# mit-han-lab/duo-attention

Measured on NVIDIA H100. Metric: decode tok/s @512K ctx (+ prefill tok/s @128K in `prefill`), Llama-3-8B, DuoAttention 50% retrieval heads, higher is better.
Workload: dtype bf16

## Files before the change

duo_attention_b200/_C.py:

```python
from __future__ import annotations

import ctypes as C
import os

_HERE = os.path.dirname(os.path.abspath(__file__))
LIB_PATH = os.environ.get("DUO_B200_LIB") or os.path.join(_HERE, "csrc", "libduo_b200.so")

DUO_OK, DUO_EINVAL, DUO_EOVERFLOW, DUO_ECUDA, DUO_EWORKSPACE = 0, -1, -2, -3, -4
DT_BF16, DT_FP16 = 0, 1
KV_SAME, KV_INT4 = 0, 1
ROPE_NONE, ROPE_HF, ROPE_FP32 = 0, 1, 2
ROPE_SKIP_Q = 0x100
DECODE_MAX_Q = 16
DECODE_MAX_Q_INT4 = 8
RAGGED_MAX_BATCH = 64

SYMBOLS = [
    "duo_layer_create", "duo_layer_destroy", "duo_workspace_bytes", "duo_rope_append", "duo_attention",
    "duo_attention_mma", "duo_decode_fused", "duo_decode_ragged", "duo_ragged_workspace_bytes",
    "duo_decode_ragged_int4", "duo_ragged_int4_workspace_bytes", "duo_layer_create_pooled", "duo_decode_ragged_pooled",
    "duo_ragged_state_advance", "duo_state_advance", "duo_state_set", "duo_stream_commit", "duo_quant_int4", "duo_dequant_int4", "duo_dequant_int4_bf16", "duo_add_rmsnorm", "duo_silu_mul",
    "duo_attention_partial", "duo_merge_partials", "duo_attention_seq", "duo_decode_fused_seq",
    "duo_attention_seq_int4", "duo_decode_fused_seq_int4",
    "duo_seqcomm_data_bytes", "duo_seqcomm_flag_bytes", "duo_seqcomm_create", "duo_seqcomm_destroy", "duo_seq_merge",
    "duo_comm_data_bytes", "duo_comm_flag_bytes", "duo_comm_create", "duo_comm_destroy", "duo_allreduce_add_rmsnorm",
    "duo_last_error_string", "duo_version",
]


class LayerDesc(C.Structure):
    _fields_ = [
        ("full_k", C.c_void_p), ("full_v", C.c_void_p), ("ring_k", C.c_void_p), ("ring_v", C.c_void_p),
        ("full_k_scale", C.c_void_p), ("full_k_zero", C.c_void_p), ("full_v_scale", C.c_void_p),
        ("full_v_zero", C.c_void_p), ("ring_k_scale", C.c_void_p), ("ring_k_zero", C.c_void_p),
        ("ring_v_scale", C.c_void_p), ("ring_v_zero", C.c_void_p),
        ("full_cap", C.c_int64),
        ("batch", C.c_int32), ("n_full", C.c_int32), ("n_stream", C.c_int32), ("group", C.c_int32),
        ("head_dim", C.c_int32), ("sink", C.c_int32), ("recent", C.c_int32), ("stage_cap", C.c_int32),
        ("dtype", C.c_int32), ("kv_format", C.c_int32),
    ]


class CacheState(C.Structure):
    _fields_ = [("full_len", C.c_int64), ("total", C.c_int64), ("lo", C.c_int64), ("device_state", C.c_void_p),
                ("seq_rank", C.c_int32), ("seq_world", C.c_int32), ("seq_block", C.c_int32), ("seq_reserved", C.c_int32)]


class SeqCommDesc(C.Structure):
    _fields_ = [("data", C.c_void_p * 8), ("flags", C.c_void_p * 8), ("local_state", C.c_void_p),
                ("rank", C.c_int32), ("world", C.c_int32), ("max_rows", C.c_int32)]


class CommDesc(C.Structure):
    _fields_ = [("data", C.c_void_p * 8), ("flags", C.c_void_p * 8), ("local_state", C.c_void_p),
# ... 29 lines not shown
        fn = getattr(lib, name)
        fn.argtypes = [vp, C.POINTER(CacheState), vp, i64, vp, i32, f32, vp, sz, vp]
        fn.restype = C.c_int
    lib.duo_decode_fused.argtypes = [vp, C.POINTER(CacheState), vp, i64, vp, vp, i32, vp, i32, f32, vp, sz, vp]
    lib.duo_decode_fused.restype = C.c_int
    for name in ("duo_decode_ragged", "duo_decode_ragged_int4"):
        fn = getattr(lib, name)
        fn.argtypes = [vp, vp, i64, vp, i64, vp, vp, i32, vp, i32, f32, vp, sz, vp]
        fn.restype = C.c_int
    lib.duo_decode_ragged_pooled.argtypes = [vp, vp, vp, i64, vp, i64, vp, vp, i32, vp, i32, f32, vp, sz, vp]
    lib.duo_decode_ragged_pooled.restype = C.c_int
    for name in ("duo_ragged_workspace_bytes", "duo_ragged_int4_workspace_bytes"):
        fn = getattr(lib, name)
        fn.argtypes = [i32, i32]
        fn.restype = sz
    lib.duo_ragged_state_advance.argtypes = [vp, i32, i32, i32, i32, vp]
    lib.duo_ragged_state_advance.restype = C.c_int
    lib.duo_state_advance.argtypes = [vp, i32, i32, i32, vp]
    lib.duo_state_advance.restype = C.c_int
    lib.duo_state_set.argtypes = [vp, i64, i64, i64, vp]
    lib.duo_state_set.restype = C.c_int
    lib.duo_stream_commit.argtypes = [vp, C.POINTER(CacheState), i32, vp]
    lib.duo_stream_commit.restype = C.c_int
    lib.duo_quant_int4.argtypes = [vp, i64, i64, vp, vp, vp, vp]
    lib.duo_quant_int4.restype = C.c_int
    for name in ("duo_dequant_int4", "duo_dequant_int4_bf16"):
        fn = getattr(lib, name)
        fn.argtypes = [vp, vp, vp, i64, vp, vp]
        fn.restype = C.c_int
    lib.duo_add_rmsnorm.argtypes = [vp, vp, vp, vp, vp, i64, i32, f32, i32, vp]
    lib.duo_add_rmsnorm.restype = C.c_int
    lib.duo_silu_mul.argtypes = [vp, vp, i64, i32, i32, vp]
    lib.duo_silu_mul.restype = C.c_int
    lib.duo_attention_partial.argtypes = [vp, i64, vp, i64, vp, vp, i32, f32, vp, sz, vp]
    lib.duo_attention_partial.restype = C.c_int
    for name in ("duo_attention_seq", "duo_attention_seq_int4"):
        fn = getattr(lib, name)
        fn.argtypes = [vp, C.POINTER(CacheState), vp, i64, vp, vp, vp, i32, f32, vp, sz, vp]
        fn.restype = C.c_int
    for name in ("duo_decode_fused_seq", "duo_decode_fused_seq_int4"):
        fn = getattr(lib, name)
        fn.argtypes = [vp, C.POINTER(CacheState), vp, i64, vp, vp, i32, vp, vp, vp, f32, vp, sz, vp]
        fn.restype = C.c_int
    lib.duo_seqcomm_data_bytes.argtypes = [i32, i32]
    lib.duo_seqcomm_data_bytes.restype = sz
    lib.duo_seqcomm_flag_bytes.argtypes = [i32, i32]
    lib.duo_seqcomm_flag_bytes.restype = sz
    lib.duo_seqcomm_create.argtypes = [C.POINTER(SeqCommDesc), C.POINTER(vp)]
    lib.duo_seqcomm_create.restype = C.c_int
    lib.duo_seqcomm_destroy.argtypes = [vp]
    lib.duo_seqcomm_destroy.restype = None
    lib.duo_seq_merge.argtypes = [vp, vp, vp, vp, i32, i32, i32, i32, vp]
    lib.duo_seq_merge.restype = C.c_int
    lib.duo_merge_partials.argtypes = [vp, vp, i32, i64, i32, i32, vp, i32, vp]
    lib.duo_merge_partials.restype = C.c_int
    lib.duo_comm_data_bytes.argtypes = [i32, i32, i32, i32]
    lib.duo_comm_data_bytes.restype = sz
    lib.duo_comm_flag_bytes.argtypes = [i32, i32]
    lib.duo_comm_flag_bytes.restype = sz
    lib.duo_comm_create.argtypes = [C.POINTER(CommDesc), C.POINTER(vp)]
    lib.duo_comm_create.restype = C.c_int
    lib.duo_comm_destroy.argtypes = [vp]
    lib.duo_comm_destroy.restype = None
    lib.duo_allreduce_add_rmsnorm.argtypes = [vp, vp, vp, vp, vp, vp, i32, f32, vp]
    lib.duo_allreduce_add_rmsnorm.restype = C.c_int
    lib.duo_last_error_string.argtypes = []
# ... 19 lines not shown
```

duo_attention_b200/csrc/api.cu:

```cuda
#include <cstdarg>
#include <cstdio>
#include <cstdlib>
#include <cstring>
#include <new>

#include "duo_common.cuh"

namespace duo {

int sm_count_current_device() {
  static int sms[64] = {0};
  int dev = 0;
  if (cudaGetDevice(&dev) != cudaSuccess) return 132;
  int& v = sms[dev & 63];
  if (v == 0) {
    int n = 132;
    if (cudaDeviceGetAttribute(&n, cudaDevAttrMultiProcessorCount, dev) != cudaSuccess || n < 1) n = 132;
    v = n;
  }
  return v;
}

static thread_local char g_err[512] = "";

// ... 35 lines not shown
                        float* part_o, float* part_lse, int q_len, float scale, void* workspace, size_t workspace_bytes,
                        cudaStream_t stream);
int launch_decode_fused(const duo_layer* L, const duo_cache_state* st, const void* qkv, long long row_stride,
                        const void* cos, const void* sin, int rope_mode, void* out, int q_len, float scale,
                        void* workspace, size_t workspace_bytes, cudaStream_t stream);
int launch_decode_fused_int4(const duo_layer* L, const duo_cache_state* st, const void* qkv, long long row_stride,
                             const void* cos, const void* sin, int rope_mode, void* out, int q_len, float scale,
                             void* workspace, size_t workspace_bytes, cudaStream_t stream);
int launch_decode_ragged(const duo_layer* L, const long long* row_state, const long long* row_geom, const void* qkv,
                         long long row_stride, const void* cos, const void* sin, int rope_mode, void* out, int q_len,
                         float scale, void* workspace, size_t workspace_bytes, cudaStream_t stream);
size_t ragged_workspace_bytes(int batch, int n_kv);
int launch_decode_ragged_int4(const duo_layer* L, const long long* row_state, const long long* row_geom,
                              const void* qkv, long long row_stride, const void* cos, const void* sin, int rope_mode,
                              void* out, int q_len, float scale, void* workspace, size_t workspace_bytes,
                              cudaStream_t stream);
size_t ragged_int4_workspace_bytes(int batch, int n_kv);
int launch_ragged_state_advance(long long* st, int batch, int n, int sink, int recent, cudaStream_t stream);
int launch_decode_fused_seq(const duo_layer* L, const duo_cache_state* st, const void* qkv, long long row_stride,
                            const void* cos, const void* sin, int rope_mode, void* out, float* part_o, float* part_lse,
                            float scale, void* workspace, size_t workspace_bytes, cudaStream_t stream);
int launch_attn_int4_seq(const duo_layer* L, const duo_cache_state* st, const void* q, long long q_row_stride,
                         void* out, float* part_o, float* part_lse, int q_len, float scale, void* workspace,
                         size_t workspace_bytes, cudaStream_t stream);
int launch_decode_fused_seq_int4(const duo_layer* L, const duo_cache_state* st, const void* qkv, long long row_stride,
                                 const void* cos, const void* sin, int rope_mode, void* out, float* part_o,
                                 float* part_lse, float scale, void* workspace, size_t workspace_bytes,
                                 cudaStream_t stream);
int launch_merge_partials(const float* o_parts, const float* lse_parts, int n_parts, long long tokens, int heads_total,
                          int heads_used, void* out, int dtype, cudaStream_t stream);
int launch_add_rmsnorm(const void* x, const void* residual, const void* weight, void* out_norm, void* out_res,
                       long long rows, int hidden, float eps, int dtype, cudaStream_t stream);
int launch_silu_mul(const void* gate_up, void* out, long long rows, int inter, int dtype, cudaStream_t stream);

typedef CUresult (*EncodeTiledFn)(CUtensorMap*, CUtensorMapDataType, cuuint32_t, void*, const cuuint64_t*,
                                  const cuuint64_t*, const cuuint32_t*, const cuuint32_t*, CUtensorMapInterleave,
                                  CUtensorMapSwizzle, CUtensorMapL2promotion, CUtensorMapFloatOOBfill);

EncodeTiledFn get_encode_fn() {
  static EncodeTiledFn fn = nullptr;
  if (fn) return fn;
  void* p = nullptr;
  cudaDriverEntryPointQueryResult qres;
  cudaError_t e = cudaGetDriverEntryPoint("cuTensorMapEncodeTiled", &p, cudaEnableDefault, &qres);
  if (e != cudaSuccess || qres != cudaDriverEntryPointSuccess || p == nullptr) {
    set_error("cudaGetDriverEntryPoint(cuTensorMapEncodeTiled) failed: %s", cudaGetErrorString(e));
    cudaGetLastError();
    return nullptr;
  }
  fn = reinterpret_cast<EncodeTiledFn>(p);
  return fn;
}

static int encode_kv_map(CUtensorMap* m, void* base, int dtype, long long slots, long long heads, int box_rows) {
  EncodeTiledFn fn = get_encode_fn();
  if (!fn) return DUO_ECUDA;
  cuuint64_t dims[3] = {(cuuint64_t)kHeadDim, (cuuint64_t)slots, (cuuint64_t)heads};
  cuuint64_t strides[2] = {(cuuint64_t)kHeadDim * 2, (cuuint64_t)slots * kHeadDim * 2};
  cuuint32_t box[3] = {64, (cuuint32_t)box_rows, 1};
  cuuint32_t estr[3] = {1, 1, 1};
  CUresult r = fn(m, dtype == DUO_DT_BF16 ? CU_TENSOR_MAP_DATA_TYPE_BFLOAT16 : CU_TENSOR_MAP_DATA_TYPE_FLOAT16, 3, base,
                  dims, strides, box, estr, CU_TENSOR_MAP_INTERLEAVE_NONE, CU_TENSOR_MAP_SWIZZLE_128B,
                  CU_TENSOR_MAP_L2_PROMOTION_L2_256B, CU_TENSOR_MAP_FLOAT_OOB_FILL_NONE);
  if (r != CUDA_SUCCESS) {
    set_error("cuTensorMapEncodeTiled failed with CUresult %d (base=%p slots=%lld heads=%lld)", (int)r, base, slots,
              heads);
// ... 509 lines not shown
}

int duo_merge_partials(const float* o_parts, const float* lse_parts, int32_t n_parts, int64_t tokens,
                       int32_t heads_total, int32_t heads_used, void* out, int32_t dtype, void* stream) {
  if (n_parts < 1 || tokens < 0 || heads_total < 1 || heads_used < 0 || heads_used > heads_total ||
      (tokens > 0 && heads_used > 0 && (!o_parts || !lse_parts || !out)) ||
      (dtype != DUO_DT_BF16 && dtype != DUO_DT_FP16)) {
    set_error("duo_merge_partials: bad argument");
    return DUO_EINVAL;
  }
  return launch_merge_partials(o_parts, lse_parts, n_parts, tokens, heads_total, heads_used, out, dtype,
                               (cudaStream_t)stream);
}

int duo_add_rmsnorm(const void* x, const void* residual, const void* weight, void* out_norm, void* out_res, int64_t rows,
                    int32_t hidden, float eps, int32_t dtype, void* stream) {
  if (rows < 0 || hidden < 8 || hidden % 8 != 0 || hidden > 16384 || (rows > 0 && (!x || !weight || !out_norm)) ||
      (dtype != DUO_DT_BF16 && dtype != DUO_DT_FP16)) {
    set_error("duo_add_rmsnorm: bad argument");
    return DUO_EINVAL;
  }
  return launch_add_rmsnorm(x, residual, weight, out_norm, out_res, rows, hidden, eps, dtype, (cudaStream_t)stream);
}

int duo_silu_mul(const void* gate_up, void* out, int64_t rows, int32_t inter, int32_t dtype, void* stream) {
  if (rows < 0 || inter < 8 || inter % 8 != 0 || (rows > 0 && (!gate_up || !out)) ||
      (dtype != DUO_DT_BF16 && dtype != DUO_DT_FP16)) {
    set_error("duo_silu_mul: bad argument");
    return DUO_EINVAL;
  }
  return launch_silu_mul(gate_up, out, rows, inter, dtype, (cudaStream_t)stream);
}

int duo_dequant_int4(const void* packed, const void* scale, const void* zero, int64_t rows, void* out, void* stream) {
  if (rows < 0 || (rows > 0 && (!packed || !scale || !zero || !out))) {
    set_error("duo_dequant_int4: bad argument");
    return DUO_EINVAL;
  }
  return launch_dequant_int4(packed, scale, zero, rows, out, (cudaStream_t)stream);
}

int duo_dequant_int4_bf16(const void* packed, const void* scale, const void* zero, int64_t rows, void* out,
                          void* stream) {
  if (rows < 0 || (rows > 0 && (!packed || !scale || !zero || !out))) {
    set_error("duo_dequant_int4_bf16: bad argument");
    return DUO_EINVAL;
  }
  return launch_dequant_int4_bf16(packed, scale, zero, rows, out, (cudaStream_t)stream);
}

}
```

duo_attention_b200/csrc/duo_common.cuh:

```cuda
#pragma once
#include <cuda.h>
#include <cuda_bf16.h>
#include <cuda_fp16.h>
#include <cuda_runtime.h>
#include <stdint.h>

#include <algorithm>

#include "../../include/duo_b200.h"

namespace duo {

constexpr int kHeadDim = 128;

void set_error(const char* fmt, ...);
int cuda_fail(cudaError_t e, const char* what);
#define DUO_CUDA_TRY(expr)                                   \
  do {                                                       \
    cudaError_t _e = (expr);                                 \
    if (_e != cudaSuccess) return ::duo::cuda_fail(_e, #expr); \
  } while (0)

struct LayerMaps {
  CUtensorMap full_k64, full_v64;
// ... 632 lines not shown
  const void* cos = nullptr;
  const void* sin = nullptr;
  int rope_mode = DUO_ROPE_NONE;
};

template <typename P>
inline void fill_fused_args(P& p, const FusedArgs& fa) {
  p.cos = fa.cos;
  p.sin = fa.sin;
  p.rope_mode = fa.rope_mode;
  p.k_off = (long long)p.n_q_heads * kHeadDim;
  p.v_off = (long long)(p.n_q_heads + p.n_full + p.n_stream) * kHeadDim;
}

struct KvMaps {
  const CUtensorMap *fk, *fv, *rk, *rv;
};
inline KvMaps kv_maps(const duo_layer* L, bool box128) {
  const LayerMaps& m = L->maps;
  const CUtensorMap* fk = box128 ? &m.full_k128 : &m.full_k64;
  const CUtensorMap* fv = box128 ? &m.full_v128 : &m.full_v64;
  const CUtensorMap* rk = box128 ? &m.ring_k128 : &m.ring_k64;
  const CUtensorMap* rv = box128 ? &m.ring_v128 : &m.ring_v64;
  return {L->has_full_maps ? fk : rk, L->has_full_maps ? fv : rv, L->has_ring_maps ? rk : fk,
          L->has_ring_maps ? rv : fv};
}

template <typename F>
inline int dispatch_dtype(int dtype, F&& f) {
  if (dtype == DUO_DT_BF16) return f(__nv_bfloat16{});
  return f(__half{});
}

}
```

duo_attention_b200/csrc/elementwise.cu:

```cuda
#include "duo_common.cuh"

namespace duo {

template <typename T>
struct EwCvt;
template <>
struct EwCvt<__nv_bfloat16> {
  __device__ static float to_f(__nv_bfloat16 v) { return __bfloat162float(v); }
  __device__ static __nv_bfloat16 from_f(float v) { return __float2bfloat16_rn(v); }
};
template <>
struct EwCvt<__half> {
  __device__ static float to_f(__half v) { return __half2float(v); }
  __device__ static __half from_f(float v) { return __float2half_rn(v); }
};

template <typename T>
struct alignas(16) Vec8 {
  T v[8];
};

template <typename T>
__global__ void __launch_bounds__(256) add_rmsnorm_kernel(const T* __restrict__ x, const T* __restrict__ residual,
                                                          const T* __restrict__ weight, T* __restrict__ out_norm,
                                                          T* __restrict__ out_res, int hidden, float eps) {
  extern __shared__ float s_row[];
  __shared__ float s_part[8];
  const long long row = blockIdx.x;
  const T* xr = x + row * hidden;
  const T* rr = residual ? residual + row * hidden : nullptr;
  float ss = 0.f;
  for (int i = threadIdx.x * 8; i < hidden; i += blockDim.x * 8) {
    Vec8<T> a = *reinterpret_cast<const Vec8<T>*>(xr + i);
    if (rr) {
      const Vec8<T> b = *reinterpret_cast<const Vec8<T>*>(rr + i);
#pragma unroll
      for (int k = 0; k < 8; ++k) a.v[k] = EwCvt<T>::from_f(EwCvt<T>::to_f(b.v[k]) + EwCvt<T>::to_f(a.v[k]));
      if (out_res) *reinterpret_cast<Vec8<T>*>(out_res + row * hidden + i) = a;
    }
#pragma unroll
    for (int k = 0; k < 8; ++k) {
      const float f = EwCvt<T>::to_f(a.v[k]);
      s_row[i + k] = f;
      ss += f * f;
    }
  }
#pragma unroll
  for (int o = 16; o > 0; o >>= 1) ss += __shfl_xor_sync(0xffffffffu, ss, o);
  if ((threadIdx.x & 31) == 0) s_part[threadIdx.x >> 5] = ss;
  __syncthreads();
  float tot = 0.f;
#pragma unroll
  for (int w = 0; w < 8; ++w) tot += (w < (int)(blockDim.x >> 5)) ? s_part[w] : 0.f;
  const float inv = rsqrtf(tot / (float)hidden + eps);
  for (int i = threadIdx.x * 8; i < hidden; i += blockDim.x * 8) {
    const Vec8<T> w = *reinterpret_cast<const Vec8<T>*>(weight + i);
    Vec8<T> o;
#pragma unroll
    for (int k = 0; k < 8; ++k) {
      const T n = EwCvt<T>::from_f(s_row[i + k] * inv);
      o.v[k] = EwCvt<T>::from_f(EwCvt<T>::to_f(w.v[k]) * EwCvt<T>::to_f(n));
    }
    *reinterpret_cast<Vec8<T>*>(out_norm + row * hidden + i) = o;
  }
}

template <typename T>
__global__ void __launch_bounds__(256) silu_mul_kernel(const T* __restrict__ gate_up, T* __restrict__ out, long long rows,
                                                       int inter) {
  const long long per_row = inter / 8;
  const long long idx = (long long)blockIdx.x * blockDim.x + threadIdx.x;
  if (idx >= rows * per_row) return;
  const long long row = idx / per_row;
  const int c = (int)(idx % per_row) * 8;
  const Vec8<T> g = *reinterpret_cast<const Vec8<T>*>(gate_up + row * 2 * inter + c);
  const Vec8<T> u = *reinterpret_cast<const Vec8<T>*>(gate_up + row * 2 * inter + inter + c);
  Vec8<T> o;
#pragma unroll
  for (int k = 0; k < 8; ++k) {
    const float gf = EwCvt<T>::to_f(g.v[k]);
    const T act = EwCvt<T>::from_f(gf / (1.0f + __expf(-gf)));
    o.v[k] = EwCvt<T>::from_f(EwCvt<T>::to_f(act) * EwCvt<T>::to_f(u.v[k]));
  }
  *reinterpret_cast<Vec8<T>*>(out + row * inter + c) = o;
}

int launch_add_rmsnorm(const void* x, const void* residual, const void* weight, void* out_norm, void* out_res,
                       long long rows, int hidden, float eps, int dtype, cudaStream_t stream) {
  if (rows == 0) return DUO_OK;
  const size_t smem = (size_t)hidden * sizeof(float);
  if (smem > 48 * 1024) {
    static unsigned long long mask_bf = 0, mask_h = 0;
    const int rc = dtype == DUO_DT_BF16 ? ensure_dyn_smem(add_rmsnorm_kernel<__nv_bfloat16>, 64 * 1024, &mask_bf)
                                        : ensure_dyn_smem(add_rmsnorm_kernel<__half>, 64 * 1024, &mask_h);
    if (rc) return rc;
  }
  if (dtype == DUO_DT_BF16) {
    add_rmsnorm_kernel<__nv_bfloat16><<<(unsigned)rows, 256, smem, stream>>>(
        (const __nv_bfloat16*)x, (const __nv_bfloat16*)residual, (const __nv_bfloat16*)weight, (__nv_bfloat16*)out_norm,
        (__nv_bfloat16*)out_res, hidden, eps);
  } else {
    add_rmsnorm_kernel<__half><<<(unsigned)rows, 256, smem, stream>>>((const __half*)x, (const __half*)residual,
                                                                      (const __half*)weight, (__half*)out_norm,
                                                                      (__half*)out_res, hidden, eps);
  }
  DUO_CUDA_TRY(cudaGetLastError());
  return DUO_OK;
}

int launch_silu_mul(const void* gate_up, void* out, long long rows, int inter, int dtype, cudaStream_t stream) {
  if (rows == 0) return DUO_OK;
  const long long n = rows * (inter / 8);
  const unsigned blocks = (unsigned)((n + 255) / 256);
  if (dtype == DUO_DT_BF16)
    silu_mul_kernel<__nv_bfloat16><<<blocks, 256, 0, stream>>>((const __nv_bfloat16*)gate_up, (__nv_bfloat16*)out, rows, inter);
  else
    silu_mul_kernel<__half><<<blocks, 256, 0, stream>>>((const __half*)gate_up, (__half*)out, rows, inter);
  DUO_CUDA_TRY(cudaGetLastError());
  return DUO_OK;
}

}
```

duo_attention_b200/ops.py:

```python
from __future__ import annotations

import torch

from . import _C

LAUNCHES = 0


def _dt(t):
    if t.dtype == torch.bfloat16:
        return _C.DT_BF16
    if t.dtype == torch.float16:
        return _C.DT_FP16
    raise ValueError(f"dtype {t.dtype} not supported (bf16 / fp16)")


def add_rmsnorm(x: torch.Tensor, residual, weight: torch.Tensor, eps: float, inplace_residual: bool = True):
    global LAUNCHES
    if not x.is_cuda:
        raise RuntimeError("duo_attention_b200 kernels need CUDA tensors (no CPU fallback)")
    hidden = x.shape[-1]
    x = x if x.is_contiguous() else x.contiguous()
    rows = x.numel() // hidden
    out = torch.empty_like(x)
    res_ptr, out_res, h = None, None, x
    if residual is not None:
        assert residual.is_contiguous() and residual.shape == x.shape and residual.dtype == x.dtype
        h = residual if inplace_residual else torch.empty_like(x)
        res_ptr, out_res = residual.data_ptr(), h.data_ptr()
    _C.check(_C.load().duo_add_rmsnorm(x.data_ptr(), res_ptr, weight.data_ptr(), out.data_ptr(), out_res, rows, hidden,
                                      float(eps), _dt(x), torch.cuda.current_stream(x.device).cuda_stream))
    LAUNCHES += 1
    return out, h


def silu_mul(gate_up: torch.Tensor):
    global LAUNCHES
    if not gate_up.is_cuda:
        raise RuntimeError("duo_attention_b200 kernels need CUDA tensors (no CPU fallback)")
    inter = gate_up.shape[-1] // 2
    gate_up = gate_up if gate_up.is_contiguous() else gate_up.contiguous()
    rows = gate_up.numel() // (2 * inter)
    out = torch.empty(*gate_up.shape[:-1], inter, dtype=gate_up.dtype, device=gate_up.device)
    _C.check(_C.load().duo_silu_mul(gate_up.data_ptr(), out.data_ptr(), rows, inter, _dt(gate_up),
                                   torch.cuda.current_stream(gate_up.device).cuda_stream))
    LAUNCHES += 1
    return out
```

duo_attention_b200/patch/hf_driver.py:

```python
from __future__ import annotations

import types
from typing import Optional

import torch
from transformers.modeling_outputs import CausalLMOutputWithPast

from .. import _C
from ..kv_cache import DuoKVCache, DuoRaggedKVCache, model_geometry


class _AttnPlan:

    def __init__(self, n_full, n_kv, group, head_dim):
        self.n_full, self.n_kv, self.group, self.head_dim = n_full, n_kv, group, head_dim
        self.wqkv = None
        self.bqkv = None


def _fuse_qkv(attn):
    plan = attn._duo_plan
    w = torch.cat([attn.q_proj.weight.data, attn.k_proj.weight.data, attn.v_proj.weight.data], dim=0).contiguous()
    nq, nk = attn.q_proj.weight.shape[0], attn.k_proj.weight.shape[0]
    attn.q_proj.weight.data = w[:nq]
    attn.k_proj.weight.data = w[nq : nq + nk]
    attn.v_proj.weight.data = w[nq + nk :]
    plan.wqkv = w
    if attn.q_proj.bias is not None:
        plan.bqkv = torch.cat([attn.q_proj.bias.data, attn.k_proj.bias.data, attn.v_proj.bias.data]).contiguous()


def _fuse_gate_up(mlp):
    w = torch.cat([mlp.gate_proj.weight.data, mlp.up_proj.weight.data], dim=0).contiguous()
    n = mlp.gate_proj.weight.shape[0]
    mlp.gate_proj.weight.data = w[:n]
    mlp.up_proj.weight.data = w[n:]
    mlp._duo_wgu = w


def _mlp_forward(mlp, x):
    from .. import ops

    w = getattr(mlp, "_duo_wgu", None)
    if w is None or w.device != x.device:
        _fuse_gate_up(mlp)
        w = mlp._duo_wgu
    return mlp.down_proj(ops.silu_mul(torch.nn.functional.linear(x, w)))


def _fusable(layer):
    m = layer.mlp
    return (all(hasattr(m, n) for n in ("gate_proj", "up_proj", "down_proj"))
            and m.gate_proj.bias is None and m.up_proj.bias is None
            and type(getattr(m, "act_fn", None)).__name__ in ("SiLU", "SiLUActivation")
            and hasattr(layer.input_layernorm, "variance_epsilon"))


def duo_attention_layer_forward(attn, hidden_states, cos, sin, kv_cache: DuoKVCache, layer_idx: int,
                                rope_mode: int = _C.ROPE_HF, project: bool = True):
    plan = attn._duo_plan
    if plan.wqkv is None or plan.wqkv.device != hidden_states.device:
        _fuse_qkv(attn)
    B, S, _ = hidden_states.shape
    qkv = torch.nn.functional.linear(hidden_states, plan.wqkv, plan.bqkv)
    out = torch.empty(B, S, plan.n_kv * plan.group, plan.head_dim, dtype=qkv.dtype, device=qkv.device)
    kv_cache.attend(layer_idx, qkv, cos, sin, rope_mode, out)
    return attn.o_proj(out.view(B, S, -1)) if project else out.view(B, S, -1)


def _tp_layer_pipelined(layer, ctx, h, next_norm, group, n_blocks):
    import torch.distributed as dist

    from .. import ops

    S = ctx.shape[1]
    step = (S + n_blocks - 1) // n_blocks
    spans = [(r, min(S, r + step)) for r in range(0, S, step)]
    ln2 = layer.post_attention_layernorm
    parts, works = [], []
    for r0, r1 in spans:
        a = layer.self_attn.o_proj(ctx[:, r0:r1])
        works.append(dist.all_reduce(a, op=dist.ReduceOp.SUM, group=group, async_op=True))
        parts.append(a)
    mparts, mworks = [], []
    for (r0, r1), a, w in zip(spans, parts, works):
        w.wait()
        x, _ = ops.add_rmsnorm(a, h[:, r0:r1], ln2.weight, ln2.variance_epsilon)
        m = _mlp_forward(layer.mlp, x)
        mworks.append(dist.all_reduce(m, op=dist.ReduceOp.SUM, group=group, async_op=True))
        mparts.append(m)
    outs = []
    for (r0, r1), m, w in zip(spans, mparts, mworks):
        w.wait()
        x, _ = ops.add_rmsnorm(m, h[:, r0:r1], next_norm.weight, next_norm.variance_epsilon)
        outs.append(x)
    return torch.cat(outs, dim=1)


def plans_head_dim(model):
    return model.model.layers[0].self_attn._duo_plan.head_dim
# ... 114 lines not shown
                x, h = ops.add_rmsnorm(a, h, ln2.weight, ln2.variance_epsilon)
            else:
                x, h = reduce_add_norm(a, h, ln2.weight, ln2.variance_epsilon)
            m = _mlp_forward(layer.mlp, x)
            if idx + 1 < len(layers):
                nxt = layers[idx + 1].input_layernorm
                x, h = reduce_add_norm(m, h, nxt.weight, nxt.variance_epsilon)
            else:
                if tp_on and comm is None:
                    m = all_reduce_sum(m, self._duo_tp_group)
                m_last, h_last = m[:, -1:, :].contiguous(), h[:, -1:, :].contiguous()
                if comm is not None:
                    x, _ = comm.add_rmsnorm(m_last, h_last, base.norm.weight, base.norm.variance_epsilon)
                else:
                    x, _ = ops.add_rmsnorm(m_last, h_last, base.norm.weight, base.norm.variance_epsilon)
        h = x
    else:
        for idx, layer in enumerate(layers):
            res = h
            x = layer.input_layernorm(h)
            x = duo_attention_layer_forward(layer.self_attn, x, cos, sin, cache, idx, rope_mode)
            if tp_on and not seq_on:
                x = all_reduce_sum(x, self._duo_tp_group)
            h = res + x
            res = h
            x = layer.post_attention_layernorm(h)
            x = layer.mlp(x)
            if tp_on:
                x = all_reduce_sum(x, self._duo_tp_group)
            h = res + x
        h = base.norm(h[:, -1:, :])
    if cache.dev_state is not None:
        cache.advance_device(S)
    logits = self.lm_head(h)
    if getattr(self, "_duo_logits_float", True):
        logits = logits.float()
    return CausalLMOutputWithPast(logits=logits, past_key_values=cache if use_cache is not False else None)


def install(model, full_attention_heads, sink_size, recent_size, logits_float=True, rope="hf"):
    from .reorder import reorder_linear_weights, reorder_full_attn_heads

    geo = model_geometry(model)
    n_kv, head_dim = geo["num_kv_heads"], geo["head_dim"]
    group = geo["num_heads"] // n_kv
    for idx, layer in enumerate(model.model.layers):
        module = layer.self_attn
        gate = torch.tensor(full_attention_heads[idx], device=geo["device"], dtype=geo["dtype"])
        reorder_linear_weights(module.q_proj, gate, group * head_dim, "out")
        reorder_linear_weights(module.k_proj, gate, head_dim, "out")
        reorder_linear_weights(module.v_proj, gate, head_dim, "out")
        reorder_linear_weights(module.o_proj, gate, group * head_dim, "in")
        gate = reorder_full_attn_heads(gate)
        module.sink_size = sink_size
        module.recent_size = recent_size
        module.register_buffer("full_attention_heads", gate)
        module._duo_plan = _AttnPlan(int((gate > 0.5).sum().item()), n_kv, group, head_dim)
    model._duo_sink = sink_size
    model._duo_recent = recent_size
    model._duo_logits_float = logits_float
    if rope not in ("hf", "flashinfer"):
        raise ValueError(f"rope must be 'hf' or 'flashinfer', got {rope!r}")
    model._duo_rope_mode = _C.ROPE_FP32 if rope == "flashinfer" else _C.ROPE_HF
    model.forward = types.MethodType(duo_causal_lm_forward, model)
    return model
```

include/duo_b200.h:

```cpp
#ifndef DUO_B200_H
#define DUO_B200_H

#include <stddef.h>
#include <stdint.h>

#ifdef __cplusplus
extern "C" {
#endif

#if defined(__GNUC__)
#define DUO_API __attribute__((visibility("default")))
#else
#define DUO_API
#endif

#define DUO_OK 0
#define DUO_EINVAL -1
#define DUO_EOVERFLOW -2
#define DUO_ECUDA -3
#define DUO_EWORKSPACE -4

#define DUO_DT_BF16 0
#define DUO_DT_FP16 1
#define DUO_KV_SAME 0
// ... 66 lines not shown
DUO_API int duo_decode_ragged_int4(const duo_layer* layer, const int64_t* row_state, int64_t max_full_len,
                                   const void* qkv, int64_t qkv_row_stride, const void* cos, const void* sin,
                                   int32_t rope_mode, void* out, int32_t q_len, float scale, void* workspace,
                                   size_t workspace_bytes, void* stream);
DUO_API size_t duo_ragged_int4_workspace_bytes(int32_t batch, int32_t n_kv_heads);
DUO_API int duo_layer_create_pooled(const duo_layer_desc* desc, int64_t pool_tokens, duo_layer** out);
DUO_API int duo_decode_ragged_pooled(const duo_layer* layer, const int64_t* row_state, const int64_t* row_geom,
                                     int64_t min_room, const void* qkv, int64_t qkv_row_stride, const void* cos,
                                     const void* sin, int32_t rope_mode, void* out, int32_t q_len, float scale,
                                     void* workspace, size_t workspace_bytes, void* stream);
DUO_API int duo_ragged_state_advance(int64_t* row_state, int32_t batch, int32_t n, int32_t sink, int32_t recent,
                                     void* stream);

DUO_API int duo_attention_mma(const duo_layer* layer, const duo_cache_state* st, const void* q, int64_t q_row_stride,
                              void* out, int32_t q_len, float scale, void* workspace, size_t workspace_bytes,
                              void* stream);

DUO_API int duo_state_advance(int64_t* device_state, int32_t n, int32_t sink, int32_t recent, void* stream);
DUO_API int duo_state_set(int64_t* device_state, int64_t full_len, int64_t total, int64_t lo, void* stream);

DUO_API int duo_stream_commit(const duo_layer* layer, const duo_cache_state* st, int32_t q_len, void* stream);

DUO_API int duo_quant_int4(const void* in, int64_t in_row_stride, int64_t rows, void* packed, void* scale,
                   void* zero, void* stream);
DUO_API int duo_dequant_int4(const void* packed, const void* scale, const void* zero, int64_t rows, void* out,
                     void* stream);
DUO_API int duo_dequant_int4_bf16(const void* packed, const void* scale, const void* zero, int64_t rows, void* out,
                                  void* stream);

DUO_API int duo_add_rmsnorm(const void* x, const void* residual, const void* weight, void* out_norm, void* out_res,
                            int64_t rows, int32_t hidden, float eps, int32_t dtype, void* stream);
DUO_API int duo_silu_mul(const void* gate_up, void* out, int64_t rows, int32_t inter, int32_t dtype, void* stream);

DUO_API int duo_attention_partial(const duo_layer* layer, int64_t n_keys, const void* q, int64_t q_row_stride,
                                  float* out_o, float* out_lse, int32_t q_len, float scale, void* workspace,
                                  size_t workspace_bytes, void* stream);
DUO_API int duo_attention_seq(const duo_layer* layer, const duo_cache_state* st, const void* q, int64_t q_row_stride,
                              void* out, float* out_o, float* out_lse, int32_t q_len, float scale, void* workspace,
                              size_t workspace_bytes, void* stream);
DUO_API int duo_decode_fused_seq(const duo_layer* layer, const duo_cache_state* st, const void* qkv, int64_t qkv_row_stride,
                                 const void* cos, const void* sin, int32_t rope_mode, void* out, float* out_o,
                                 float* out_lse, float scale, void* workspace, size_t workspace_bytes, void* stream);
DUO_API int duo_attention_seq_int4(const duo_layer* layer, const duo_cache_state* st, const void* q,
                                   int64_t q_row_stride, void* out, float* out_o, float* out_lse, int32_t q_len,
                                   float scale, void* workspace, size_t workspace_bytes, void* stream);
DUO_API int duo_decode_fused_seq_int4(const duo_layer* layer, const duo_cache_state* st, const void* qkv,
                                      int64_t qkv_row_stride, const void* cos, const void* sin, int32_t rope_mode,
                                      void* out, float* out_o, float* out_lse, float scale, void* workspace,
                                      size_t workspace_bytes, void* stream);
DUO_API int duo_merge_partials(const float* o_parts, const float* lse_parts, int32_t n_parts, int64_t tokens,
                               int32_t heads_total, int32_t heads_used, void* out, int32_t dtype, void* stream);

typedef struct duo_comm duo_comm;
typedef struct duo_comm_desc {
  void* data[8];
  void* flags[8];
  void* local_state;
  int32_t rank, world;
  int32_t hidden;
  int32_t max_rows;
  int32_t dtype;
} duo_comm_desc;
DUO_API size_t duo_comm_data_bytes(int32_t world, int32_t hidden, int32_t max_rows, int32_t dtype);
DUO_API size_t duo_comm_flag_bytes(int32_t world, int32_t max_rows);
DUO_API int duo_comm_create(const duo_comm_desc* desc, duo_comm** out);
DUO_API void duo_comm_destroy(duo_comm* comm);
// ... 27 lines not shown
```

Before: 56.53.

## Add custom decode GEMV kernel with fused SiLU-mul and PDL launches

Adds a tensor-core GEMV kernel for single-row decode inputs that streams weights through a multi-stage cp.async ring, optionally fuses SiLU-mul into the down projection's input, and optionally writes fp32 logits directly. The QKV, o_proj, MLP and lm_head projections route through it when the input is a single row. Both it and add_rmsnorm are launched with programmatic dependent launch, so a kernel's weight prefetch can overlap the tail of the previous kernel. The aim is to cut cuBLAS overhead, separate silu_mul and cast launches, and launch gaps in weight-bandwidth-bound decode. The risk is that the hand-written GEMV reaches lower bandwidth than cuBLAS on the large lm_head or MLP shapes.

```diff
diff --git a/duo_attention_b200/_C.py b/duo_attention_b200/_C.py
--- a/duo_attention_b200/_C.py
+++ b/duo_attention_b200/_C.py
@@ -14,12 +14,14 @@
 DECODE_MAX_Q = 16
 DECODE_MAX_Q_INT4 = 8
 RAGGED_MAX_BATCH = 64
+GEMV_MAX_ROWS = 8
+GEMV_SILU_MUL, GEMV_F32_OUT = 0x1, 0x2
 
 SYMBOLS = [
     "duo_layer_create", "duo_layer_destroy", "duo_workspace_bytes", "duo_rope_append", "duo_attention",
     "duo_attention_mma", "duo_decode_fused", "duo_decode_ragged", "duo_ragged_workspace_bytes",
     "duo_decode_ragged_int4", "duo_ragged_int4_workspace_bytes", "duo_layer_create_pooled", "duo_decode_ragged_pooled",
-    "duo_ragged_state_advance", "duo_state_advance", "duo_state_set", "duo_stream_commit", "duo_quant_int4", "duo_dequant_int4", "duo_dequant_int4_bf16", "duo_add_rmsnorm", "duo_silu_mul",
+    "duo_ragged_state_advance", "duo_state_advance", "duo_state_set", "duo_stream_commit", "duo_quant_int4", "duo_dequant_int4", "duo_dequant_int4_bf16", "duo_add_rmsnorm", "duo_silu_mul", "duo_gemv",
     "duo_attention_partial", "duo_merge_partials", "duo_attention_seq", "duo_decode_fused_seq",
     "duo_attention_seq_int4", "duo_decode_fused_seq_int4",
     "duo_seqcomm_data_bytes", "duo_seqcomm_flag_bytes", "duo_seqcomm_create", "duo_seqcomm_destroy", "duo_seq_merge",
@@ -115,6 +117,8 @@
     lib.duo_add_rmsnorm.restype = C.c_int
     lib.duo_silu_mul.argtypes = [vp, vp, i64, i32, i32, vp]
     lib.duo_silu_mul.restype = C.c_int
+    lib.duo_gemv.argtypes = [vp, vp, vp, vp, i32, i64, i32, i32, i32, vp]
+    lib.duo_gemv.restype = C.c_int
     lib.duo_attention_partial.argtypes = [vp, i64, vp, i64, vp, vp, i32, f32, vp, sz, vp]
     lib.duo_attention_partial.restype = C.c_int
     for name in ("duo_attention_seq", "duo_attention_seq_int4"):
diff --git a/duo_attention_b200/csrc/api.cu b/duo_attention_b200/csrc/api.cu
--- a/duo_attention_b200/csrc/api.cu
+++ b/duo_attention_b200/csrc/api.cu
@@ -91,6 +91,8 @@
 int launch_add_rmsnorm(const void* x, const void* residual, const void* weight, void* out_norm, void* out_res,
                        long long rows, int hidden, float eps, int dtype, cudaStream_t stream);
 int launch_silu_mul(const void* gate_up, void* out, long long rows, int inter, int dtype, cudaStream_t stream);
+int launch_gemv(const void* x, const void* w, const void* bias, void* y, int rows, int n, int k, int flags, int dtype,
+                cudaStream_t stream);
 
 typedef CUresult (*EncodeTiledFn)(CUtensorMap*, CUtensorMapDataType, cuuint32_t, void*, const cuuint64_t*,
                                   const cuuint64_t*, const cuuint32_t*, const cuuint32_t*, CUtensorMapInterleave,
@@ -666,6 +668,27 @@
   return launch_silu_mul(gate_up, out, rows, inter, dtype, (cudaStream_t)stream);
 }
 
+int duo_gemv(const void* x, const void* w, const void* bias, void* y, int32_t rows, int64_t n, int32_t k,
+             int32_t flags, int32_t dtype, void* stream) {
+  if (!x || !w || !y) {
+    set_error("duo_gemv: null buffer");
+    return DUO_EINVAL;
+  }
+  if (rows < 1 || rows > DUO_GEMV_MAX_ROWS || n < 1 || n > INT32_MAX || k < 8 || k % 8 != 0 ||
+      (flags & ~(DUO_GEMV_SILU_MUL | DUO_GEMV_F32_OUT)) || (dtype != DUO_DT_BF16 && dtype != DUO_DT_FP16)) {
+    set_error("duo_gemv: bad argument (rows %d of 1..%d, n %lld, k %d a positive multiple of 8, flags 0x%x, dtype %d)",
+              rows, DUO_GEMV_MAX_ROWS, (long long)n, k, flags, dtype);
+    return DUO_EINVAL;
+  }
+  if ((reinterpret_cast<uintptr_t>(x) | reinterpret_cast<uintptr_t>(w)) % 16 != 0 ||
+      reinterpret_cast<uintptr_t>(bias) % 2 != 0 ||
+      reinterpret_cast<uintptr_t>(y) % ((flags & DUO_GEMV_F32_OUT) ? 4 : 2) != 0) {
+    set_error("duo_gemv: x and w must be 16-byte aligned, bias and y element-aligned");
+    return DUO_EINVAL;
+  }
+  return launch_gemv(x, w, bias, y, rows, (int)n, k, flags, dtype, (cudaStream_t)stream);
+}
+
 int duo_dequant_int4(const void* packed, const void* scale, const void* zero, int64_t rows, void* out, void* stream) {
   if (rows < 0 || (rows > 0 && (!packed || !scale || !zero || !out))) {
     set_error("duo_dequant_int4: bad argument");
diff --git a/duo_attention_b200/csrc/duo_common.cuh b/duo_attention_b200/csrc/duo_common.cuh
--- a/duo_attention_b200/csrc/duo_common.cuh
+++ b/duo_attention_b200/csrc/duo_common.cuh
@@ -688,4 +688,24 @@
   return f(__half{});
 }
 
-}
+__device__ __forceinline__ void griddep_wait() { asm volatile("griddepcontrol.wait;" ::: "memory"); }
+__device__ __forceinline__ void griddep_launch_dependents() { asm volatile("griddepcontrol.launch_dependents;" ::: "memory"); }
+
+template <typename... Params, typename... Args>
+inline int launch_pdl(void (*kern)(Params...), dim3 grid, dim3 block, size_t smem, cudaStream_t stream,
+                      Args... args) {
+  cudaLaunchAttribute attr[1];
+  attr[0].id = cudaLaunchAttributeProgrammaticStreamSerialization;
+  attr[0].val.programmaticStreamSerializationAllowed = 1;
+  cudaLaunchConfig_t cfg = {};
+  cfg.gridDim = grid;
+  cfg.blockDim = block;
+  cfg.dynamicSmemBytes = smem;
+  cfg.stream = stream;
+  cfg.attrs = attr;
+  cfg.numAttrs = 1;
+  DUO_CUDA_TRY(cudaLaunchKernelEx(&cfg, kern, static_cast<Params>(args)...));
+  return DUO_OK;
+}
+
+}
diff --git a/duo_attention_b200/csrc/elementwise.cu b/duo_attention_b200/csrc/elementwise.cu
--- a/duo_attention_b200/csrc/elementwise.cu
+++ b/duo_attention_b200/csrc/elementwise.cu
@@ -1,24 +1,6 @@
-#include "duo_common.cuh"
+#include "elementwise.cuh"
 
 namespace duo {
-
-template <typename T>
-struct EwCvt;
-template <>
-struct EwCvt<__nv_bfloat16> {
-  __device__ static float to_f(__nv_bfloat16 v) { return __bfloat162float(v); }
-  __device__ static __nv_bfloat16 from_f(float v) { return __float2bfloat16_rn(v); }
-};
-template <>
-struct EwCvt<__half> {
-  __device__ static float to_f(__half v) { return __half2float(v); }
-  __device__ static __half from_f(float v) { return __float2half_rn(v); }
-};
-
-template <typename T>
-struct alignas(16) Vec8 {
-  T v[8];
-};
 
 template <typename T>
 __global__ void __launch_bounds__(256) add_rmsnorm_kernel(const T* __restrict__ x, const T* __restrict__ residual,
@@ -26,6 +8,8 @@
                                                           T* __restrict__ out_res, int hidden, float eps) {
   extern __shared__ float s_row[];
   __shared__ float s_part[8];
+  griddep_wait();
+  griddep_launch_dependents();
   const long long row = blockIdx.x;
   const T* xr = x + row * hidden;
   const T* rr = residual ? residual + row * hidden : nullptr;
@@ -77,11 +61,7 @@
   const Vec8<T> u = *reinterpret_cast<const Vec8<T>*>(gate_up + row * 2 * inter + inter + c);
   Vec8<T> o;
 #pragma unroll
-  for (int k = 0; k < 8; ++k) {
-    const float gf = EwCvt<T>::to_f(g.v[k]);
-    const T act = EwCvt<T>::from_f(gf / (1.0f + __expf(-gf)));
-    o.v[k] = EwCvt<T>::from_f(EwCvt<T>::to_f(act) * EwCvt<T>::to_f(u.v[k]));
-  }
+  for (int k = 0; k < 8; ++k) o.v[k] = silu_mul_value(g.v[k], u.v[k]);
   *reinterpret_cast<Vec8<T>*>(out + row * inter + c) = o;
 }
 
@@ -95,17 +75,11 @@
                                         : ensure_dyn_smem(add_rmsnorm_kernel<__half>, 64 * 1024, &mask_h);
     if (rc) return rc;
   }
-  if (dtype == DUO_DT_BF16) {
-    add_rmsnorm_kernel<__nv_bfloat16><<<(unsigned)rows, 256, smem, stream>>>(
-        (const __nv_bfloat16*)x, (const __nv_bfloat16*)residual, (const __nv_bfloat16*)weight, (__nv_bfloat16*)out_norm,
-        (__nv_bfloat16*)out_res, hidden, eps);
-  } else {
-    add_rmsnorm_kernel<__half><<<(unsigned)rows, 256, smem, stream>>>((const __half*)x, (const __half*)residual,
-                                                                      (const __half*)weight, (__half*)out_norm,
-                                                                      (__half*)out_res, hidden, eps);
-  }
-  DUO_CUDA_TRY(cudaGetLastError());
-  return DUO_OK;
+  return dispatch_dtype(dtype, [&](auto t) {
+    using T = decltype(t);
+    return launch_pdl(add_rmsnorm_kernel<T>, dim3((unsigned)rows), dim3(256), smem, stream, (const T*)x,
+                      (const T*)residual, (const T*)weight, (T*)out_norm, (T*)out_res, hidden, eps);
+  });
 }
 
 int launch_silu_mul(const void* gate_up, void* out, long long rows, int inter, int dtype, cudaStream_t stream) {
diff --git a/duo_attention_b200/csrc/elementwise.cuh b/duo_attention_b200/csrc/elementwise.cuh
--- /dev/null
+++ b/duo_attention_b200/csrc/elementwise.cuh
@@ -0,0 +1,31 @@
+#pragma once
+#include "duo_common.cuh"
+
+namespace duo {
+
+template <typename T>
+struct EwCvt;
+template <>
+struct EwCvt<__nv_bfloat16> {
+  __device__ static float to_f(__nv_bfloat16 v) { return __bfloat162float(v); }
+  __device__ static __nv_bfloat16 from_f(float v) { return __float2bfloat16_rn(v); }
+};
+template <>
+struct EwCvt<__half> {
+  __device__ static float to_f(__half v) { return __half2float(v); }
+  __device__ static __half from_f(float v) { return __float2half_rn(v); }
+};
+
+template <typename T>
+struct alignas(16) Vec8 {
+  T v[8];
+};
+
+template <typename T>
+__device__ __forceinline__ T silu_mul_value(T g, T u) {
+  const float gf = EwCvt<T>::to_f(g);
+  const T act = EwCvt<T>::from_f(gf / (1.0f + __expf(-gf)));
+  return EwCvt<T>::from_f(EwCvt<T>::to_f(act) * EwCvt<T>::to_f(u));
+}
+
+}
diff --git a/duo_attention_b200/csrc/gemv.cu b/duo_attention_b200/csrc/gemv.cu
--- /dev/null
+++ b/duo_attention_b200/csrc/gemv.cu
@@ -0,0 +1,194 @@
+#include "elementwise.cuh"
+
+namespace duo {
+
+namespace {
+
+constexpr int kWarps = 2;
+constexpr int kStripRows = 16;
+constexpr int kStageK = 64;
+constexpr int kStages = 8;
+constexpr int kRowBytes = kStageK * 2 + 16;
+constexpr int kStageBytes = kStripRows * kRowBytes;
+constexpr int kRingBytes = kWarps * kStages * kStageBytes;
+constexpr int kXBytes = 32 * 1024;
+constexpr int kSmemBytes = kRingBytes + kXBytes;
+
+__device__ __forceinline__ void cp_async16(uint32_t dst, const void* src, bool valid) {
+  asm volatile("cp.async.cg.shared.global [%0], [%1], 16, %2;" ::"r"(dst), "l"(src), "r"(valid ? 16 : 0) : "memory");
+}
+__device__ __forceinline__ void cp_async_commit() { asm volatile("cp.async.commit_group;" ::: "memory"); }
+template <int N>
+__device__ __forceinline__ void cp_async_wait() {
+  asm volatile("cp.async.wait_group %0;" ::"n"(N) : "memory");
+}
+
+template <typename T>
+__device__ __forceinline__ void mma16816(float (&c)[4], const uint32_t (&a)[4], uint32_t b0, uint32_t b1);
+template <>
+__device__ __forceinline__ void mma16816<__nv_bfloat16>(float (&c)[4], const uint32_t (&a)[4], uint32_t b0,
+                                                        uint32_t b1) {
+  asm volatile("mma.sync.aligned.m16n8k16.row.col.f32.bf16.bf16.f32 {%0,%1,%2,%3}, {%4,%5,%6,%7}, {%8,%9}, "
+               "{%0,%1,%2,%3};"
+               : "+f"(c[0]), "+f"(c[1]), "+f"(c[2]), "+f"(c[3])
+               : "r"(a[0]), "r"(a[1]), "r"(a[2]), "r"(a[3]), "r"(b0), "r"(b1));
+}
+template <>
+__device__ __forceinline__ void mma16816<__half>(float (&c)[4], const uint32_t (&a)[4], uint32_t b0, uint32_t b1) {
+  asm volatile("mma.sync.aligned.m16n8k16.row.col.f32.f16.f16.f32 {%0,%1,%2,%3}, {%4,%5,%6,%7}, {%8,%9}, "
+               "{%0,%1,%2,%3};"
+               : "+f"(c[0]), "+f"(c[1]), "+f"(c[2]), "+f"(c[3])
+               : "r"(a[0]), "r"(a[1]), "r"(a[2]), "r"(a[3]), "r"(b0), "r"(b1));
+}
+
+template <typename T, bool SILU>
+__device__ __forceinline__ uint32_t x_pair(const T* x, long long xk, int k_len, int r, int k) {
+  const T* p = x + r * xk + k;
+  if constexpr (SILU) {
+    const T* u = p + k_len;
+    T o[2] = {silu_mul_value(p[0], u[0]), silu_mul_value(p[1], u[1])};
+    return *reinterpret_cast<const uint32_t*>(o);
+  } else {
+    return *reinterpret_cast<const uint32_t*>(p);
+  }
+}
+
+template <typename T, bool SILU>
+__global__ void __launch_bounds__(kWarps * 32)
+    gemv_kernel(const T* __restrict__ x, const T* __restrict__ w, const T* __restrict__ bias, void* __restrict__ y,
+                int rows, int n, int k, int splits, int f32_out) {
+  extern __shared__ __align__(16) unsigned char smem[];
+  __shared__ float s_part[kWarps][kStripRows][8];
+  const int lane = threadIdx.x & 31, warp = threadIdx.x >> 5;
+  const int split = warp % splits;
+  const int r0 = (blockIdx.x * (kWarps / splits) + warp / splits) * kStripRows;
+  const bool active = r0 < n;
+  const int k_len = k / splits;
+  const int k_lo = split * k_len;
+  const int steps = (k_len + kStageK - 1) / kStageK;
+  const uint32_t ring = smem_u32(smem + warp * kStages * kStageBytes);
+
+  auto issue = [&](int s) {
+    if (s < steps) {
+      const uint32_t dst = ring + (s % kStages) * kStageBytes;
+      const int kc = k_lo + s * kStageK + (lane & 7) * 8;
+#pragma unroll
+      for (int i = 0; i < 4; ++i) {
+        const int rr = (lane >> 3) + 4 * i;
+        const bool ok = active && r0 + rr < n && kc < k_lo + k_len;
+        cp_async16(dst + rr * kRowBytes + (lane & 7) * 16, ok ? w + (long long)(r0 + rr) * k + kc : w, ok);
+      }
+    }
+    cp_async_commit();
+  };
+#pragma unroll 1
+  for (int s = 0; s < kStages - 1; ++s) issue(s);
+
+  griddep_wait();
+  griddep_launch_dependents();
+
+  T* xs = reinterpret_cast<T*>(smem + kRingBytes);
+  const bool staged = (long long)rows * k * 2 <= kXBytes;
+  if (staged) {
+    for (int i = threadIdx.x; i < rows * (k >> 3); i += kWarps * 32) {
+      const int r = i / (k >> 3), kc = (i % (k >> 3)) * 8;
+      Vec8<T> v;
+      if constexpr (SILU) {
+        const Vec8<T> gv = *reinterpret_cast<const Vec8<T>*>(x + r * 2ll * k + kc);
+        const Vec8<T> uv = *reinterpret_cast<const Vec8<T>*>(x + r * 2ll * k + k + kc);
+#pragma unroll
+        for (int e = 0; e < 8; ++e) v.v[e] = silu_mul_value(gv.v[e], uv.v[e]);
+      } else {
+        v = *reinterpret_cast<const Vec8<T>*>(x + r * (long long)k + kc);
+      }
+      *reinterpret_cast<Vec8<T>*>(xs + r * k + kc) = v;
+    }
+  }
+  __syncthreads();
+
+  const int g = lane >> 2, t = lane & 3;
+  float c[4] = {0.f, 0.f, 0.f, 0.f};
+  const long long xk = SILU ? 2ll * k : (long long)k;
+#pragma unroll 1
+  for (int s = 0; s < steps; ++s) {
+    cp_async_wait<kStages - 2>();
+    __syncwarp();
+    issue(s + kStages - 1);
+    const uint32_t stage = ring + (s % kStages) * kStageBytes;
+#pragma unroll
+    for (int kk = 0; kk < kStageK / 16; ++kk) {
+      const int kb = s * kStageK + kk * 16;
+      if (kb >= k_len) break;
+      uint32_t a[4];
+      asm volatile("ldmatrix.sync.aligned.m8n8.x4.shared.b16 {%0,%1,%2,%3}, [%4];"
+                   : "=r"(a[0]), "=r"(a[1]), "=r"(a[2]), "=r"(a[3])
+                   : "r"(stage + (lane & 15) * kRowBytes + (kk * 16 + (lane >> 4) * 8) * 2));
+      uint32_t b0 = 0u, b1 = 0u;
+      if (g < rows) {
+        const int kx = k_lo + kb + 2 * t;
+        if (staged) {
+          b0 = *reinterpret_cast<const uint32_t*>(xs + g * k + kx);
+          if (kb + 8 < k_len) b1 = *reinterpret_cast<const uint32_t*>(xs + g * k + kx + 8);
+        } else {
+          b0 = x_pair<T, SILU>(x, xk, k, g, kx);
+          if (kb + 8 < k_len) b1 = x_pair<T, SILU>(x, xk, k, g, kx + 8);
+        }
+      }
+      mma16816<T>(c, a, b0, b1);
+    }
+  }
+  cp_async_wait<0>();
+
+  if (splits > 1 && split == 1) {
+    s_part[warp][g][2 * t] = c[0];
+    s_part[warp][g][2 * t + 1] = c[1];
+    s_part[warp][g + 8][2 * t] = c[2];
+    s_part[warp][g + 8][2 * t + 1] = c[3];
+  }
+  __syncthreads();
+  if (!active || split != 0) return;
+  if (splits > 1) {
+    c[0] += s_part[warp + 1][g][2 * t];
+    c[1] += s_part[warp + 1][g][2 * t + 1];
+    c[2] += s_part[warp + 1][g + 8][2 * t];
+    c[3] += s_part[warp + 1][g + 8][2 * t + 1];
+  }
+#pragma unroll
+  for (int i = 0; i < 4; ++i) {
+    const int ar = 2 * t + (i & 1), wr = r0 + g + (i >> 1) * 8;
+    if (ar < rows && wr < n) {
+      float v = c[i];
+      if (bias) v += EwCvt<T>::to_f(bias[wr]);
+      const T out = EwCvt<T>::from_f(v);
+      const long long at = (long long)ar * n + wr;
+      if (f32_out)
+        static_cast<float*>(y)[at] = EwCvt<T>::to_f(out);
+      else
+        static_cast<T*>(y)[at] = out;
+    }
+  }
+}
+
+}
+
+int launch_gemv(const void* x, const void* w, const void* bias, void* y, int rows, int n, int k, int flags, int dtype,
+                cudaStream_t stream) {
+  const int splits = (n <= 4096 && k % 16 == 0) ? 2 : 1;
+  const int strips_per_cta = kWarps / splits;
+  const dim3 grid((unsigned)(((n + kStripRows - 1) / kStripRows + strips_per_cta - 1) / strips_per_cta));
+  const int f32 = (flags & DUO_GEMV_F32_OUT) ? 1 : 0;
+  return dispatch_dtype(dtype, [&](auto tag) {
+    using T = decltype(tag);
+    static unsigned long long mask[2] = {0, 0};
+    if (flags & DUO_GEMV_SILU_MUL) {
+      if (int rc = ensure_dyn_smem(gemv_kernel<T, true>, kSmemBytes, &mask[0])) return rc;
+      return launch_pdl(gemv_kernel<T, true>, grid, dim3(kWarps * 32), kSmemBytes, stream, (const T*)x, (const T*)w,
+                        (const T*)bias, y, rows, n, k, splits, f32);
+    }
+    if (int rc = ensure_dyn_smem(gemv_kernel<T, false>, kSmemBytes, &mask[1])) return rc;
+    return launch_pdl(gemv_kernel<T, false>, grid, dim3(kWarps * 32), kSmemBytes, stream, (const T*)x, (const T*)w,
+                      (const T*)bias, y, rows, n, k, splits, f32);
+  });
+}
+
+}
diff --git a/duo_attention_b200/ops.py b/duo_attention_b200/ops.py
--- a/duo_attention_b200/ops.py
+++ b/duo_attention_b200/ops.py
@@ -34,6 +34,34 @@
     return out, h
 
 
+GEMV_MODEL_ROWS = 1
+
+
+def gemv_fits(x: torch.Tensor, w: torch.Tensor) -> bool:
+    return (x.is_cuda and x.dtype in (torch.bfloat16, torch.float16) and w.dtype == x.dtype
+            and x.numel() <= GEMV_MODEL_ROWS * x.shape[-1] and x.shape[-1] % 8 == 0)
+
+
+def gemv(x: torch.Tensor, w: torch.Tensor, bias=None, silu_mul: bool = False, out_float: bool = False):
+    global LAUNCHES
+    if not x.is_cuda:
+        raise RuntimeError("duo_attention_b200 kernels need CUDA tensors (no CPU fallback)")
+    if not w.is_contiguous() or (bias is not None and not bias.is_contiguous()):
+        raise ValueError("gemv: the weight and bias must be contiguous")
+    x = x if x.is_contiguous() else x.contiguous()
+    k = x.shape[-1] // 2 if silu_mul else x.shape[-1]
+    rows = x.numel() // x.shape[-1]
+    n = w.shape[0]
+    if w.dim() != 2 or w.shape[1] != k or w.dtype != x.dtype or (bias is not None and bias.shape != (n,)):
+        raise ValueError(f"gemv: weight {tuple(w.shape)} {w.dtype} does not match input rows of {k} {x.dtype}")
+    y = torch.empty(*x.shape[:-1], n, dtype=torch.float32 if out_float else x.dtype, device=x.device)
+    flags = (_C.GEMV_SILU_MUL if silu_mul else 0) | (_C.GEMV_F32_OUT if out_float else 0)
+    _C.check(_C.load().duo_gemv(x.data_ptr(), w.data_ptr(), bias.data_ptr() if bias is not None else None,
+                                y.data_ptr(), rows, n, k, flags, _dt(x), torch.cuda.current_stream(x.device).cuda_stream))
+    LAUNCHES += 1
+    return y
+
+
 def silu_mul(gate_up: torch.Tensor):
     global LAUNCHES
     if not gate_up.is_cuda:
diff --git a/duo_attention_b200/patch/hf_driver.py b/duo_attention_b200/patch/hf_driver.py
--- a/duo_attention_b200/patch/hf_driver.py
+++ b/duo_attention_b200/patch/hf_driver.py
@@ -28,6 +28,12 @@
     plan.wqkv = w
     if attn.q_proj.bias is not None:
         plan.bqkv = torch.cat([attn.q_proj.bias.data, attn.k_proj.bias.data, attn.v_proj.bias.data]).contiguous()
+    _weights_written(w)
+
+
+def _weights_written(w):
+    if w.is_cuda:
+        torch.cuda.current_stream(w.device).synchronize()
 
 
 def _fuse_gate_up(mlp):
@@ -36,6 +42,13 @@
     mlp.gate_proj.weight.data = w[:n]
     mlp.up_proj.weight.data = w[n:]
     mlp._duo_wgu = w
+    _weights_written(w)
+
+
+def _linear(x, w, b=None):
+    from .. import ops
+
+    return ops.gemv(x, w, b) if ops.gemv_fits(x, w) else torch.nn.functional.linear(x, w, b)
 
 
 def _mlp_forward(mlp, x):
@@ -45,6 +58,8 @@
     if w is None or w.device != x.device:
         _fuse_gate_up(mlp)
         w = mlp._duo_wgu
+    if ops.gemv_fits(x, w):
+        return ops.gemv(ops.gemv(x, w), mlp.down_proj.weight, mlp.down_proj.bias, silu_mul=True)
     return mlp.down_proj(ops.silu_mul(torch.nn.functional.linear(x, w)))
 
 
@@ -62,10 +77,10 @@
     if plan.wqkv is None or plan.wqkv.device != hidden_states.device:
         _fuse_qkv(attn)
     B, S, _ = hidden_states.shape
-    qkv = torch.nn.functional.linear(hidden_states, plan.wqkv, plan.bqkv)
+    qkv = _linear(hidden_states, plan.wqkv, plan.bqkv)
     out = torch.empty(B, S, plan.n_kv * plan.group, plan.head_dim, dtype=qkv.dtype, device=qkv.device)
     kv_cache.attend(layer_idx, qkv, cos, sin, rope_mode, out)
-    return attn.o_proj(out.view(B, S, -1)) if project else out.view(B, S, -1)
+    return _linear(out.view(B, S, -1), attn.o_proj.weight, attn.o_proj.bias) if project else out.view(B, S, -1)
 
 
 def _tp_layer_pipelined(layer, ctx, h, next_norm, group, n_blocks):
@@ -246,9 +261,15 @@
         h = base.norm(h[:, -1:, :])
     if cache.dev_state is not None:
         cache.advance_device(S)
-    logits = self.lm_head(h)
-    if getattr(self, "_duo_logits_float", True):
-        logits = logits.float()
+    from .. import ops
+
+    logits_float = getattr(self, "_duo_logits_float", True)
+    if ops.gemv_fits(h, self.lm_head.weight):
+        logits = ops.gemv(h, self.lm_head.weight, self.lm_head.bias, out_float=logits_float)
+    else:
+        logits = self.lm_head(h)
+        if logits_float:
+            logits = logits.float()
     return CausalLMOutputWithPast(logits=logits, past_key_values=cache if use_cache is not False else None)
 
 
diff --git a/include/duo_b200.h b/include/duo_b200.h
--- a/include/duo_b200.h
+++ b/include/duo_b200.h
@@ -122,6 +122,12 @@
                             int64_t rows, int32_t hidden, float eps, int32_t dtype, void* stream);
 DUO_API int duo_silu_mul(const void* gate_up, void* out, int64_t rows, int32_t inter, int32_t dtype, void* stream);
 
+#define DUO_GEMV_MAX_ROWS 8
+#define DUO_GEMV_SILU_MUL 0x1
+#define DUO_GEMV_F32_OUT 0x2
+DUO_API int duo_gemv(const void* x, const void* w, const void* bias, void* y, int32_t rows, int64_t n, int32_t k,
+                     int32_t flags, int32_t dtype, void* stream);
+
 DUO_API int duo_attention_partial(const duo_layer* layer, int64_t n_keys, const void* q, int64_t q_row_stride,
                                   float* out_o, float* out_lse, int32_t q_len, float scale, void* workspace,
                                   size_t workspace_bytes, void* stream);
```

Result: slower. 52.05, median of 6 (-7.9%).
